# ToyotaResearchInstitute/idto

Measured on AMD Instinct MI355X. Metric: Gauss-Newton iters/sec (grad+Hessian+solve), mini_cheetah N=40, higher is better.
Workload: dtype f64; 1 GPU; mini_cheetah (nq=19, nv=18, 9 contact pairs), horizon N=40, dt=0.05, forward differences, one Gauss-Newton iteration per step; parallelism=single GPU

## Files before the change

idto_amd/csrc/fd_kernel.h:

```cpp
#pragma once

#include "batch.h"
#include "id_eval.h"
#include "id_fast.h"

namespace idto_dev {

struct DevProblem {
  int N;
  double dt;
  const double* v_init;
  const double* q_nom;
  const double* v_nom;
  const double* Qq;
  const double* Qv;
  const double* R;
  const double* Qfq;
  const double* Qfv;
  const double* Qq0; const double* Qv0; const double* R0; const double* Qfq0; const double* Qfv0;
};

__host__ __device__ __forceinline__ DevProblem at_problem(DevProblem P, size_t o) {
  P.v_init = at_problem(P.v_init, o); P.q_nom = at_problem(P.q_nom, o); P.v_nom = at_problem(P.v_nom, o);
  P.Qq = at_problem(P.Qq, o); P.Qv = at_problem(P.Qv, o); P.R = at_problem(P.R, o); P.Qfq = at_problem(P.Qfq, o);
// ... 86 lines not shown
  }
  __syncthreads();
}

IDTO_DEV double velocity_row(const DevModel& M, const double* N, const double* qa, const double* qb, double dt, int r) {
  double acc = N[r] * (qa[0] - qb[0]);
  for (int c = 1; c < M.nq; ++c) acc += N[c * M.nv + r] * (qa[c] - qb[c]);
  return acc / dt;
}
IDTO_DEV void velocity_block(const DevModel& M, const double* N, const double* qa, const double* qb, double dt,
                             double* vout, int tid, int nthreads) {
  for (int r = tid; r < M.nv; r += nthreads) vout[r] = velocity_row(M, N, qa, qb, dt, r);
}

IDTO_DEV double asm_dot(const double* A, const double* B, int nv) {
  const double2* A2 = reinterpret_cast<const double2*>(A);
  const double2* B2 = reinterpret_cast<const double2*>(B);
  double2 a = A2[0], b = B2[0];
  double acc = a.x * b.x;
  if (nv > 1) acc = acc + a.y * b.y;
  const int np = nv >> 1;
#pragma unroll 4
  for (int m = 1; m < np; ++m) {
    a = A2[m]; b = B2[m];
    acc = acc + a.x * b.x;
    acc = acc + a.y * b.y;
  }
  if ((nv & 1) && nv > 1) acc = acc + A[nv - 1] * B[nv - 1];
  return acc;
}
template <int U>
IDTO_DEV void asm_dot_n(const double* const (&A)[U], const double* const (&B)[U], int nv, double (&acc)[U]) {
  const int np = nv >> 1;
#pragma unroll
  for (int u = 0; u < U; ++u) {
    const double2 a = reinterpret_cast<const double2*>(A[u])[0], b = reinterpret_cast<const double2*>(B[u])[0];
    acc[u] = a.x * b.x;
    if (nv > 1) acc[u] = acc[u] + a.y * b.y;
  }
#pragma unroll 2
  for (int m = 1; m < np; ++m) {
#pragma unroll
    for (int u = 0; u < U; ++u) {
      const double2 a = reinterpret_cast<const double2*>(A[u])[m], b = reinterpret_cast<const double2*>(B[u])[m];
      acc[u] = acc[u] + a.x * b.x;
      acc[u] = acc[u] + a.y * b.y;
    }
  }
  if ((nv & 1) && nv > 1) {
#pragma unroll
    for (int u = 0; u < U; ++u) acc[u] = acc[u] + A[u][nv - 1] * B[u][nv - 1];
  }
}
template <int TB>
IDTO_DEV void asm_dot_tile(const double* const (&A)[TB], const double* const (&B)[TB], int nv, double (&acc)[TB][TB]) {
  const int np = nv >> 1;
  double2 a[TB], b[TB];
#pragma unroll
  for (int u = 0; u < TB; ++u) {
    a[u] = reinterpret_cast<const double2*>(A[u])[0];
    b[u] = reinterpret_cast<const double2*>(B[u])[0];
  }
#pragma unroll
  for (int ur = 0; ur < TB; ++ur)
#pragma unroll
    for (int uc = 0; uc < TB; ++uc) {
      acc[ur][uc] = a[ur].x * b[uc].x;
      if (nv > 1) acc[ur][uc] = acc[ur][uc] + a[ur].y * b[uc].y;
    }
  double2 an[TB], bn[TB];
  if (np > 1) {
#pragma unroll
    for (int u = 0; u < TB; ++u) {
      an[u] = reinterpret_cast<const double2*>(A[u])[1];
      bn[u] = reinterpret_cast<const double2*>(B[u])[1];
    }
  }
  for (int m = 1; m < np; ++m) {
#pragma unroll
    for (int u = 0; u < TB; ++u) { a[u] = an[u]; b[u] = bn[u]; }
    const int mn = (m + 1 < np) ? m + 1 : m;
#pragma unroll
    for (int u = 0; u < TB; ++u) {
      an[u] = reinterpret_cast<const double2*>(A[u])[mn];
      bn[u] = reinterpret_cast<const double2*>(B[u])[mn];
    }
#pragma unroll
    for (int ur = 0; ur < TB; ++ur)
#pragma unroll
      for (int uc = 0; uc < TB; ++uc) {
        acc[ur][uc] = acc[ur][uc] + a[ur].x * b[uc].x;
        acc[ur][uc] = acc[ur][uc] + a[ur].y * b[uc].y;
      }
  }
  if ((nv & 1) && nv > 1) {
#pragma unroll
    for (int ur = 0; ur < TB; ++ur)
#pragma unroll
      for (int uc = 0; uc < TB; ++uc) acc[ur][uc] = acc[ur][uc] + A[ur][nv - 1] * B[uc][nv - 1];
  }
}

__host__ __device__ inline int asm_terms_stride(int nq) { return 6 * nq * nq + 3 * nq + ((3 * nq) & 1); }

template <int SHAPE> struct FastShape {
  static constexpr TreeShape T = tree_shape(SHAPE);
  static constexpr int MAXC = T.MAXC, NP = T.NP, CJ = T.CJ, J0 = T.J0, K0 = T.K0, W2 = T.W2, GS = T.GS;
};
__host__ __device__ inline int fd_xch_doubles(int nxb, int threads, int npaths, int nstem = 0) {
  return (threads / npaths) * xch_eval_doubles(nxb, nstem);
}

template <int MAXC, int SHAPE = 0>
IDTO_DEV void fd_body(const DevModel& M, const DevContact& cp, const DevProblem& P, const double* __restrict__ q,
                      double* __restrict__ slab, int slab_stride, double* __restrict__ v_out,
                      double* __restrict__ a_out, double* __restrict__ nplus_out, const int k, int mode,
                      int stop_after, int echunk, double* __restrict__ terms) {
  extern __shared__ double lds[];
  constexpr bool FAST = SHAPE != 0 && SHAPE != SHAPE_XCH && SHAPE != SHAPE_STEM;
  const int tid = threadIdx.x, nt = blockDim.x;
  if (stop_after == 10) return;
#ifdef IDTO_FD_STAMPS
  long long st_arr[16] = {0, 0, 0, 0, 0, 0, 0, 0, 0, 0, 0, 0, 0, 0, 0, 0};
  long long* idto_fd_st = (tid == 0 || tid == IDTO_FD_STAMP_TID) ? st_arr : nullptr;
#endif
  FD_STAMP(0);
  const int nq = M.nq, nv = M.nv, K = M.npaths;
  const int bsz = nv * nq;
  const double dt = P.dt;

  const bool central = mode >= 2;
  const int NM = (mode == 2) ? 2 : ((mode == 3) ? 4 : 1);
  const int nP = (mode >= 1) ? NM * nq : 0;
  const int nT = (mode >= 1) ? NM * nq : 0;
  const int nM = (mode == 1) ? nv : (central ? NM * nq : 0);
  const int E = 1 + nP + nT + nM;

  double* qm1 = lds;
  double* q0 = qm1 + nq;
  double* q1 = q0 + nq;
  double* N0 = q1 + nq;
  double* N1 = N0 + bsz;
  double* v0 = N1 + bsz;
  double* v1 = v0 + nv;
  double* a0 = v1 + nv;
  double* edq = a0 + nv;
  const int EC = (echunk < E) ? echunk : E;
  double* edv = edq + E;
  double* eda = edv + E;
  double* etau = eda + E;
  double* eq = etau + E * nv;
  double* ev = eq + EC * nq;
  double* ea = ev + EC * nv;
  double* edump = ea + EC * nv;
  double* mblob = edump + nv;
  const int blob_lo = FAST ? M.fast_lo : 0, blob_n = FAST ? M.fast_n : M.blob_n;
  int* colinfo = reinterpret_cast<int*>(mblob + blob_n + (blob_n & 1));
  const int nvp = (nv + 1) & ~1, psz = nvp * nq;
  double* rec = reinterpret_cast<double*>(colinfo + nq + (nq & 1));
  rec += (rec - lds) & 1;
  double* xch = rec + (terms ? 6 * psz + nvp : 0);

  const bool sparse = M.nfloat == 0 || (M.nfloat > 0 && nt >= 128);
  const int ql = tid & 63, qcfg = tid >> 6;
  const bool quat_lane = sparse && M.nfloat > 0 && qcfg < 2 && ql >= 48 && ql < 60;
  double qf0[4];
  {
    const double* qq = q + (size_t)(k + (qcfg & 1)) * nq + (M.nfloat > 0 ? M.float_qs[0] : 0);
#pragma unroll
    for (int i = 0; i < 4; ++i) qf0[i] = qq[i];
  }
  double* wr = rec + 6 * psz;
  constexpr int BU = 8;
  double breg[BU];
#pragma unroll
  for (int u = 0; u < BU; ++u) {
    const int i = tid + u * nt;
    breg[u] = (i < blob_n) ? M.blob[blob_lo + i] : 0.0;
  }
  const bool qrow = tid < nq;
  const double g_qm1 = (qrow && k > 0) ? q[(k - 1) * nq + tid] : 0.0;
  const double g_q0 = qrow ? q[k * nq + tid] : 0.0, g_q1 = qrow ? q[(k + 1) * nq + tid] : 0.0;
  const double g_wr = (terms && mode != 0 && tid < nv) ? P.R[tid * nv + tid] : 0.0;
  const double g_nc0 = (sparse && tid < bsz) ? M.nplus_const[tid] : 0.0;
  const double g_nc1 = (sparse && tid + nt < bsz) ? M.nplus_const[tid + nt] : 0.0;
  const int g_ci = (sparse && qrow) ? M.colinfo[tid] : 0;
  const int rowinfo_r = (sparse && tid < nv) ? M.rowinfo[tid] : 0;
  asm volatile("" : "+v"(qf0[0]), "+v"(qf0[1]), "+v"(qf0[2]), "+v"(qf0[3]));
#pragma unroll
  for (int u = 0; u < BU; ++u) {
    const int i = tid + u * nt;
    if (i < blob_n) mblob[i] = breg[u];
  }
  for (int i = tid + BU * nt; i < blob_n; i += nt) mblob[i] = M.blob[blob_lo + i];
  if (qrow) { qm1[tid] = g_qm1; q0[tid] = g_q0; q1[tid] = g_q1; }
  for (int i = tid + nt; i < nq; i += nt) {
    qm1[i] = (k > 0) ? q[(k - 1) * nq + i] : 0.0;
    q0[i] = q[k * nq + i];
    q1[i] = q[(k + 1) * nq + i];
  }
  if (terms && mode != 0) {
    if (tid < nv) wr[tid] = g_wr;
    for (int l = tid + nt; l < nv; l += nt) wr[l] = P.R[l * nv + l];
  }
  if (sparse) {
    if (tid < bsz && g_nc0 == g_nc0) { N0[tid] = g_nc0; N1[tid] = g_nc0; }
    if (tid + nt < bsz && g_nc1 == g_nc1) { N0[tid + nt] = g_nc1; N1[tid + nt] = g_nc1; }
    for (int i = tid + 2 * nt; i < bsz; i += nt) {
      const double cst = M.nplus_const[i];
      if (cst == cst) { N0[i] = cst; N1[i] = cst; }
    }
    if (qrow) colinfo[tid] = g_ci;
    for (int i = tid + nt; i < nq; i += nt) colinfo[i] = M.colinfo[i];
    if (quat_lane) {
      const int e = ql - 48, r = e >> 2, c = e & 3;
      double* Nout = qcfg ? N1 : N0;
      for (int f = 0; f < M.nfloat; ++f) {
        const int qs = M.float_qs[f], vs = M.float_vs[f];
        double qq[4];
#pragma unroll
        for (int i = 0; i < 4; ++i) qq[i] = (f == 0) ? qf0[i] : q[(size_t)(k + qcfg) * nq + qs + i];
        const double nrm = __builtin_sqrt(((qq[0] * qq[0] + qq[1] * qq[1]) + qq[2] * qq[2]) + qq[3] * qq[3]);
        const double t0 = qq[0] / nrm, t1 = qq[1] / nrm, t2 = qq[2] / nrm, t3 = qq[3] / nrm;
        const double w2 = 2.0 * t0, x2 = 2.0 * t1, y2 = 2.0 * t2, z2 = 2.0 * t3;
        const double l0 = (r == 0) ? -x2 : ((r == 1) ? -y2 : -z2);
// ... 149 lines not shown
    using FS = FastShape<SHAPE>;
    FastTab FT;
    FT.body = Ml.f_body; FT.cbody = Ml.f_cbody; FT.pairs = Ml.f_pairs; FT.seg = Ml.f_seg; FT.maxpp = Ml.f_maxpp;
    FT.gslots = Ml.gslots; FT.gcommon = Ml.gcommon;
    const int grp = tid / FS::NP, path = tid % FS::NP;
    for (int e0 = 0; e0 < ce; e0 += groups) {
      const int el = (e0 == 0) ? grp : e0 + (groups - 1 - grp);
      if (el < ce) {
        const bool full = central || c0 + el < 1 + nP + nT;
        if (own_inputs) {
          InFwd in;
          in.q1 = q1; in.v1 = v1; in.a0 = a0; in.N1 = N1; in.N0 = N0; in.nv = nv;
          in.kind = (el == 0) ? 0 : ((el < 1 + nP) ? 1 : ((el < 1 + nP + nT) ? 2 : 3));
          in.col = (el == 0) ? 0 : ((el < 1 + nP) ? el - 1 : ((el < 1 + nP + nT) ? el - 1 - nP : el - 1 - nP - nT));
          in.dq = edq[el];
          in.sdv = (in.kind == 2) ? -edv[el] : ((in.kind == 1) ? edv[el] : 0.0);
          in.sda = (in.kind == 2) ? -eda[el] : ((in.kind == 1) ? eda[el] : 0.0);
          in.keep = (in.kind == 3) ? 0ull : ~0ull;
          in.keep0 = (in.kind == 2) ? ~0ull : 0ull;
          id_eval_fast<FS::MAXC, FS::NP, FS::CJ, FS::J0, FS::K0, FS::W2, FS::GS>(FT, Ml.gravity, cp, path, full, in, etau + el * nv
#ifdef IDTO_FD_STAMPS
                                                                 , (e0 == 0) ? idto_fd_st : nullptr
#endif
          );
        } else {
          InLds in;
          in.q = eq + el * nq; in.v = ev + el * nv; in.a = ea + el * nv;
          id_eval_fast<FS::MAXC, FS::NP, FS::CJ, FS::J0, FS::K0, FS::W2, FS::GS>(FT, Ml.gravity, cp, path, full, in, etau + (c0 + el) * nv);
        }
      }
    }
    if (late_outputs && tid >= nt - 64) trajectory_outputs(tid - (nt - 64), 64);
  } else {
  for (int e0 = 0; e0 < ce; e0 += groups) {
    const int el = e0 + tid / K;
    const int path = tid % K;
    const int ee = (el < ce) ? el : 0;
    const bool full = central || c0 + ee < 1 + nP + nT;
    double* tau_dst = (el < ce) ? etau + (c0 + ee) * nv : edump;
    if constexpr (SHAPE == SHAPE_STEM)
      id_eval<MAXC, true, true>(Ml, cp, path, full, eq + ee * nq, ev + ee * nv, ea + ee * nv, tau_dst,
                                xch + (tid / K) * xch_eval_doubles(Ml.nxb, Ml.nstem));
    else if constexpr (SHAPE == SHAPE_XCH)
      id_eval<MAXC, true>(Ml, cp, path, full, eq + ee * nq, ev + ee * nv, ea + ee * nv, tau_dst, xch + (tid / K) * Ml.nxb * XREC);
    else
      id_eval<MAXC>(Ml, cp, path, full, eq + ee * nq, ev + ee * nv, ea + ee * nv, tau_dst);
  }
  }
  __syncthreads();
  }

  FD_STAMP(12);
  if (stop_after == 3) return;
  double* sl = slab + (size_t)k * slab_stride;
  double* Mk = sl;
  double* Tk = sl + bsz;
  double* Pk = sl + 2 * bsz;
  double* tauk = sl + 3 * bsz;
  for (int r = tid; r < nv; r += nt) tauk[r] = etau[r];
  if (mode == 1) {
    const double sc = 1 / dt / dt;
    const double* Mcols = etau + (1 + nP + nT) * nv;
    const double fillM = (k == 0) ? __builtin_nan("") : 0.0;
    constexpr int RU = 2;
    for (int base = tid; base < bsz; base += RU * nt) {
      int ii[RU], rr[RU], j0[RU], cnt[RU];
      bool ok[RU];
      double tp[RU], tt[RU], t0[RU], dqp[RU], dqt[RU], w[RU], mc[RU][3], n0[RU][3];
#pragma unroll
      for (int u = 0; u < RU; ++u) {
        const int idx = base + u * nt;
        ok[u] = idx < bsz;
        const int id = ok[u] ? idx : 0;
        ii[u] = id / nv; rr[u] = id - ii[u] * nv;
        const int ci = colinfo[ii[u]];
        j0[u] = ci & 0xffff; cnt[u] = ci >> 16;
        tp[u] = etau[(1 + ii[u]) * nv + rr[u]]; tt[u] = etau[(1 + nP + ii[u]) * nv + rr[u]]; t0[u] = etau[rr[u]];
        dqp[u] = edq[1 + ii[u]]; dqt[u] = edq[1 + nP + ii[u]];
        w[u] = terms ? wr[rr[u]] : 0.0;
#pragma unroll
        for (int t = 0; t < 3; ++t) {
          const int j = (t < cnt[u]) ? j0[u] + t : j0[u];
          mc[u][t] = Mcols[j * nv + rr[u]];
          n0[u][t] = N0[ii[u] * nv + j];
        }
      }
#pragma unroll
      for (int u = 0; u < RU; ++u) {
        if (!ok[u]) continue;
        const int idx = base + u * nt, i = ii[u], r = rr[u];
        const double pv = (tp[u] - t0[u]) / dqp[u];
        const double tv = (k >= 1) ? (tt[u] - t0[u]) / dqt[u] : 0.0;
        double acc = (sc * mc[u][0]) * n0[u][0];
        if (cnt[u] > 1) acc += (sc * mc[u][1]) * n0[u][1];
        if (cnt[u] > 2) acc += (sc * mc[u][2]) * n0[u][2];
        const double mv = (k >= 2) ? acc : fillM;
        Pk[idx] = pv;
        Tk[idx] = tv;
        Mk[idx] = mv;
        if (terms) {
          const double mr = (k >= 2) ? acc : 0.0;
          rec[i * nvp + r] = pv; rec[psz + i * nvp + r] = tv; rec[2 * psz + i * nvp + r] = mr;
          rec[3 * psz + i * nvp + r] = pv * w[u]; rec[4 * psz + i * nvp + r] = tv * w[u]; rec[5 * psz + i * nvp + r] = mr * w[u];
          if (r == nv - 1 && nvp > nv) {
            rec[3 * psz + i * nvp + nv] = 0.0; rec[4 * psz + i * nvp + nv] = 0.0; rec[5 * psz + i * nvp + nv] = 0.0;
          }
        }
      }
    }
  } else if (central) {
    for (int idx = tid; idx < 3 * bsz; idx += nt) {
      const int g = idx / bsz, rem = idx - g * bsz, i = rem / nv, r = rem - i * nv;
      const int e0 = 1 + (g * NM) * nq + i;
      const double dq = edq[e0];
      const double tp = etau[e0 * nv + r], tm = etau[(e0 + nq) * nv + r];
      double d;
      if (mode == 2) {
        d = 0.5 * (tp - tm) / dq;
      } else {
        const double tpp = etau[(e0 + 2 * nq) * nv + r], tmm = etau[(e0 + 3 * nq) * nv + r];
        d = 2.0 / 3.0 * (tp - tm) / dq - 1.0 / 12.0 * (tpp - tmm) / dq;
      }
      const double val = (g == 0) ? d : ((g == 1) ? ((k >= 1) ? d : 0.0) : ((k >= 2) ? d : ((k == 0) ? __builtin_nan("") : 0.0)));
      if (g == 0) Pk[rem] = val;
      else if (g == 1) Tk[rem] = val;
      else Mk[rem] = val;
      if (terms) {
        const double rv = (g == 2 && k < 2) ? 0.0 : val;
        rec[g * psz + i * nvp + r] = rv;
        rec[(3 + g) * psz + i * nvp + r] = rv * wr[r];
        if (r == nv - 1 && nvp > nv) rec[(3 + g) * psz + i * nvp + nv] = 0.0;
      }
    }
  }
  if (!terms || mode == 0 || stop_after == 4) return;
  FD_STAMP(13);
  __syncthreads();
  if (stop_after == 5) return;
  const int qq = nq * nq, ts = asm_terms_stride(nq);
  double* stage = terms + (size_t)k * ts;
  constexpr int TB = 3;
  const int nb = (nq + TB - 1) / TB, ntt = nb * (nb + 1) / 2, nbb = nb * nb, ntiles = 3 * ntt + 3 * nbb;
  const float inb = 1.0f / (float)nb;
  for (int tile = tid; tile < ntiles; tile += nt) {
    if (stop_after == 6 && tile >= 3 * ntt) break;
    int xa, sb, tr, tc, ob;
    const bool lower = tile < 3 * ntt;
    if (lower) {
      const int which = (tile >= ntt) + (tile >= 2 * ntt);
      int rem = tile - which * ntt;
      tc = 0;
      while (rem >= nb - tc) { rem -= nb - tc; ++tc; }
      tr = tc + rem;
      xa = which; sb = which; ob = which * qq;
    } else {
      const int it = tile - 3 * ntt, which = (it >= nbb) + (it >= 2 * nbb), e = it - which * nbb;
      tc = (int)(((float)e + 0.5f) * inb);
      tr = e - tc * nb;
      xa = (which == 1) ? 1 : 0; sb = (which == 0) ? 1 : 2; ob = (3 + which) * qq;
    }
    const double* A[TB];
    const double* B[TB];
#pragma unroll
    for (int u = 0; u < TB; ++u) {
      const int r = tr * TB + u, c = tc * TB + u;
      A[u] = rec + (3 + xa) * psz + (r < nq ? r : nq - 1) * nvp;
      B[u] = rec + sb * psz + (c < nq ? c : nq - 1) * nvp;
    }
    double acc[TB][TB];
    asm_dot_tile<TB>(A, B, nv, acc);
#pragma unroll
    for (int ur = 0; ur < TB; ++ur)
#pragma unroll
      for (int uc = 0; uc < TB; ++uc) {
        const int r = tr * TB + ur, c = tc * TB + uc;
        if (r < nq && c < nq && (!lower || r >= c)) stage[ob + c * nq + r] = acc[ur][uc];
      }
  }
  if (stop_after != 7)
    for (int it = nt - 1 - tid; it < 3 * nq; it += nt) {
      const int which = (it >= nq) + (it >= 2 * nq), j = it - which * nq;
      const double* J = rec + which * psz + j * nvp;
      double acc = (etau[0] * wr[0]) * J[0];
      for (int r = 1; r < nv; ++r) acc += (etau[r] * wr[r]) * J[r];
      stage[6 * qq + which * nq + j] = acc;
    }
  FD_STAMP(14);
  FD_STAMP(15);
#ifdef IDTO_FD_STAMPS
  if (idto_fd_st && k == 1)
    for (int i = 0; i < 16; ++i) nplus_out[(size_t)(k + 1) * bsz + (tid == 0 ? 0 : 16) + i] = (double)(st_arr[i] - st_arr[0]);
#endif
}

template <int MAXC, int SHAPE = 0>
__global__ void __launch_bounds__(256) fd_kernel(DevModel M, DevContact cp, DevProblem P, const double* __restrict__ q,
                          double* __restrict__ slab, int slab_stride, double* __restrict__ v_out,
                          double* __restrict__ a_out, double* __restrict__ nplus_out, int k_begin, int mode,
                          int stop_after, int echunk, size_t pstride, double* __restrict__ terms, AltSel alt) {
  const size_t o = (size_t)blockIdx.y * pstride;
  const size_t w = o + (size_t)alt_offset(alt, o);
  fd_body<MAXC, SHAPE>(M, cp, at_problem(P, o), at_problem(q, o), at_problem(slab, w), slab_stride, at_problem(v_out, w),
                       at_problem(a_out, w), at_problem(nplus_out, w), k_begin + (int)blockIdx.x, mode, stop_after, echunk,
                       terms ? at_problem(terms, w) : nullptr);
}


}
```

idto_amd/csrc/host/model_tables.cc:

```cpp
#include "model_tables.h"

#include <algorithm>
#include <cmath>
#include <cstring>
#include <limits>

#include "model_layout.h"

namespace idto_host {
namespace {
using namespace idto_dev;

int Refuse(std::string* err, const char* why) {
  *err = why;
  return -1;
}

bool IdentityRotation(const double* X) {
  bool ident = true;
  for (int e = 0; e < 9; ++e) ident &= (X[e] == ((e % 4 == 0) ? 1.0 : 0.0));
  return ident;
}

int CheckGeometry(const idto_model_t* m, std::string* err) {
// ... 188 lines not shown
  std::vector<int> colinfo, rowinfo;
  int nfloat = 0, float_qs[4] = {0, 0, 0, 0}, float_vs[4] = {0, 0, 0, 0};
};
NPlus BuildNPlus(const idto_model_t* m) {
  const int nq = m->nq, nv = m->nv;
  NPlus n;
  n.constant.assign((size_t)nv * nq, 0.0);
  n.colinfo.assign(nq, 0);
  n.rowinfo.assign(nv, 0);
  auto one = [&](int q, int v) { n.constant[(size_t)q * nv + v] = 1.0; n.colinfo[q] = v | 1 << 16; n.rowinfo[v] = q | 1 << 16; };
  for (int b = 0; b < m->nbodies; ++b) {
    const int qs = m->qstart[b], vs = m->vstart[b], jt = m->jtype[b];
    if (jt == IDTO_JOINT_REVOLUTE || jt == IDTO_JOINT_PRISMATIC) {
      one(qs, vs);
    } else if (jt == IDTO_JOINT_PLANAR) {
      for (int k = 0; k < 3; ++k) one(qs + k, vs + k);
    } else {
      for (int r = 0; r < 3; ++r)
        for (int cq = 0; cq < 4; ++cq) n.constant[(size_t)(qs + cq) * nv + vs + r] = std::numeric_limits<double>::quiet_NaN();
      for (int k = 0; k < 4; ++k) n.colinfo[qs + k] = vs | 3 << 16;
      for (int r = 0; r < 3; ++r) n.rowinfo[vs + r] = qs | 4 << 16;
      for (int k = 0; k < 3; ++k) one(qs + 4 + k, vs + 3 + k);
      if (n.nfloat >= 0 && n.nfloat < 4) { n.float_qs[n.nfloat] = qs; n.float_vs[n.nfloat] = vs; ++n.nfloat; }
      else n.nfloat = -1;
    }
  }
  return n;
}

struct FastShapeOf {
  int shape = 0;
  int w2 = -1;
};
FastShapeOf RecogniseShape(const idto_model_t* m, const Stem& stem, const Star& star, bool shared, bool capsules) {
  const int K = m->npaths, cbody = m->common_body, cj = cbody >= 0 ? m->jtype[cbody] : -1;
  FastShapeOf f;
  bool ok = !(cbody >= 0 && cj != IDTO_JOINT_FLOATING) && !shared && stem.n() <= 1 && !capsules;
  for (int p = 0; p < K; ++p) ok = ok && star.nchain[p] == star.maxc;
  int j0 = -1, k0 = -1;
  for (int p = 0; p < K && ok; ++p)
    for (int s = 0; s < star.maxc; ++s) {
      const int jt = m->jtype[star.chain[star.at(p, s)]], kd = star.pkind[star.at(p, s)];
      if (s == 0) {
        if (p == 0) { j0 = jt; k0 = kd; }
        if (jt != j0 || kd != k0) ok = false;
      } else if (jt == IDTO_JOINT_REVOLUTE && kd == PK_WORLD && K == 1 && f.w2 < 0) {
        f.w2 = s;
      } else if (jt != IDTO_JOINT_REVOLUTE || kd != PK_PREV) {
        ok = false;
      }
    }
  for (int s = 1; s <= kNumTreeShapes && ok; ++s) {
    const TreeShape& t = kTreeShapes[s - 1];
    if (star.maxc == t.MAXC && K == t.NP && cj == t.CJ && j0 == t.J0 && k0 == t.K0 && f.w2 == t.W2 && (t.GS || star.all_gravity))
      f.shape = s;
  }
  return f;
}

struct FastOrder {
  std::vector<std::vector<int>> order;
  std::vector<int> seg;
};
FastOrder OrderFastPairs(const idto_model_t* m, const Star& star, const PairLists& l, FastShapeOf* f) {
  const int K = m->npaths, maxc = star.maxc, w2 = f->w2;
  const std::vector<int>&sa = l.sa, &sb = l.sb;
  FastOrder o;
  o.order.resize(K);
  o.seg.assign((size_t)K * (maxc + 2), 0);
  for (int p = 0; p < K && f->shape; ++p) {
    const int* first = l.path_pairs.data() + (size_t)p * l.maxpp;
    const std::vector<int> mine(first, first + l.path_npairs[p]);
    int lo_chain_common = 1 << 30, hi_chain_common = -1, last_slot = -1;
    for (int pi : mine) {
      const int nchainb = (sa[pi] >= 0) + (sb[pi] >= 0);
      if (nchainb > 1) {
        bool fine = w2 >= 0 && std::min(sa[pi], sb[pi]) == w2 - 1 && std::max(sa[pi], sb[pi]) == w2;
        for (int pj : mine) fine = fine && (pj == pi || (sa[pj] != w2 - 1 && sb[pj] != w2 - 1));
        if (!fine) { f->shape = 0; break; }
        continue;
      }
      if (nchainb == 1 && (sa[pi] == -1 || sb[pi] == -1)) {
        const int sl = std::max(sa[pi], sb[pi]);
        if (sl < last_slot) { f->shape = 0; break; }
        last_slot = sl;
        lo_chain_common = std::min(lo_chain_common, pi);
        hi_chain_common = std::max(hi_chain_common, pi);
      }
    }
    if (!f->shape) break;
    std::vector<std::vector<int>> groups(maxc + 2);
    for (int pi : mine) {
      const int sl = std::max(sa[pi], sb[pi]);
      if (sl >= 0) { groups[1 + sl].push_back(pi); continue; }
      const bool touches_common = sa[pi] == -1 || sb[pi] == -1;
      if (!touches_common || (sa[pi] == -1 && sb[pi] == -1)) { f->shape = 0; break; }
      if (pi < lo_chain_common) groups[0].push_back(pi);
      else if (pi > hi_chain_common) groups[maxc + 1].push_back(pi);
      else { f->shape = 0; break; }
    }
    if (!f->shape) break;
    for (int gi = 0; gi < maxc + 2; ++gi) {
      o.seg[(size_t)p * (maxc + 2) + gi] = (int)o.order[p].size() | ((int)groups[gi].size() << 16);
      for (int pi : groups[gi]) o.order[p].push_back(pi);
    }
  }
  return o;
// ... 125 lines not shown
```

idto_amd/csrc/id_fast.h:

```cpp
#pragma once

#include "id_eval.h"

#ifdef IDTO_FD_STAMPS
#ifndef IDTO_FD_STAMP_TID
#define IDTO_FD_STAMP_TID 192
#endif
#define FD_STAMP(i) do { __builtin_amdgcn_sched_barrier(0); asm volatile("" ::: "memory"); if (idto_fd_st) idto_fd_st[i] = (long long)__builtin_readcyclecounter(); asm volatile("" ::: "memory"); __builtin_amdgcn_sched_barrier(0); } while (0)
#else
#define FD_STAMP(i) do { } while (0)
#endif

namespace idto_dev {

template <int CTRL>
IDTO_DEV double quad_perm(double x) {
  int lo = __double2loint(x), hi = __double2hiint(x);
  lo = __builtin_amdgcn_update_dpp(0, lo, CTRL, 0xf, 0xf, true);
  hi = __builtin_amdgcn_update_dpp(0, hi, CTRL, 0xf, 0xf, true);
  return __hiloint2double(hi, lo);
}
template <int NP>
IDTO_DEV V3 tree_sum_fast(V3 v) {
  if (NP >= 2) {
    v.x = v.x + quad_perm<0xB1>(v.x); v.y = v.y + quad_perm<0xB1>(v.y); v.z = v.z + quad_perm<0xB1>(v.z);
  }
  if (NP >= 4) {
    v.x = v.x + quad_perm<0x4E>(v.x); v.y = v.y + quad_perm<0x4E>(v.y); v.z = v.z + quad_perm<0x4E>(v.z);
  }
  if (NP >= 8) {
    v.x = xor_add(v.x, 4); v.y = xor_add(v.y, 4); v.z = xor_add(v.z, 4);
  }
  return v;
}

IDTO_DEV const double* lds_launder(const double* p) {
  typedef __attribute__((address_space(3))) const double lds_cdouble;
  unsigned a = (unsigned)(size_t)(lds_cdouble*)p;
  asm volatile("" : "+v"(a));
  return (const double*)(lds_cdouble*)(size_t)a;
}

IDTO_DEV void pin(V3& a) { asm volatile("" : "+v"(a.x), "+v"(a.y), "+v"(a.z)); }

enum { FB_PREFETCH = FB_INERTIA + 6 };
IDTO_DEV void prefetch_record(const double* rec, double (&rc)[FB_PREFETCH]) {
#ifdef IDTO_FAST_NO_PREFETCH
#pragma unroll
  for (int i = 0; i < FB_PREFETCH; ++i) rc[i] = rec[i];
#else
  typedef __attribute__((address_space(3))) const volatile double lds_cvdouble;
  lds_cvdouble* p = (lds_cvdouble*)rec;
#pragma unroll
  for (int i = 0; i < FB_PREFETCH; ++i) rc[i] = p[i];
#endif
}

struct ParentKin {
  M3 R;
  V3 p, w, v, al, a;
// ... 397 lines not shown
```

idto_amd/csrc/idto_hip.hip:

```cpp
#include <hip/hip_runtime.h>
#include <rccl/rccl.h>
#include <dlfcn.h>

#include <atomic>
#include <chrono>
#include <cmath>
#include <cstdio>
#include <cstdlib>
#include <cstring>
#include <initializer_list>
#include <limits>
#include <memory>
#include <mutex>
#include <type_traits>
#include <utility>
#include <thread>
#include <string>
#include <vector>

#include "idto_hip.h"
#include "kernels.h"
#include "fd_launch.h"
#include "penta_ldl.h"
#include "fused.h"
// ... 390 lines not shown
      HIP_OK(hipStreamSynchronize(c->stream));
      TRACE("hip: problem upload done (one copy + wait)");
    }
  }
  auto is_diag = [](const double* W, int n) {
    for (int c2 = 0; c2 < n; ++c2)
      for (int r = 0; r < n; ++r)
        if (r != c2 && W[(size_t)c2 * n + r] != 0.0) return false;
    return true;
  };
  const bool diag = is_diag(p->Qq, nq) && is_diag(p->Qv, nv) && is_diag(p->R, nv) && is_diag(p->Qf_q, nq) &&
                    is_diag(p->Qf_v, nv);
  if ((int)c->prob_diag.size() != c->batch) c->prob_diag.assign((size_t)c->batch, 0);
  c->prob_diag[(size_t)pb] = diag ? 1 : 0;
  c->weights_diagonal = true;
  for (char d : c->prob_diag) c->weights_diagonal = c->weights_diagonal && d;
  DevProblem& P = c->P;
  P.N = N; P.dt = dt; P.v_init = c->d_vinit; P.q_nom = c->d_qnom; P.v_nom = c->d_vnom;
  P.Qq = c->d_w[0]; P.Qv = c->d_w[1]; P.R = c->d_w[2]; P.Qfq = c->d_w[3]; P.Qfv = c->d_w[4];
  P.Qq0 = c->d_w[5]; P.Qv0 = c->d_w[6]; P.R0 = c->d_w[7]; P.Qfq0 = c->d_w[8]; P.Qfv0 = c->d_w[9];
  return 0;
}

int UploadModel(idto_hip_ctx* c, const idto_model_t* m, const idto_host::ModelTables& t) {
  double* bd = nullptr;
  if (Upload(c, t.blob.data(), t.blob.size(), &bd)) return -2;
  const int* bi = reinterpret_cast<const int*>(bd);
  DevModel& M = c->M;
  M.blob = bd; M.blob_n = (int)t.blob.size();
#define X(name) M.name = bd + t.at.name;
  IDTO_MODEL_DOUBLE_TABLES(X)
#undef X
#define X(name) M.name = bi + t.at.name;
  IDTO_MODEL_INT_TABLES(X)
#undef X
  M.nb = m->nbodies; M.nq = m->nq; M.nv = m->nv; M.npaths = m->npaths; M.common_body = m->common_body;
  M.ngeoms = m->ngeoms; M.npairs = m->npairs; M.maxpp = t.maxpp;
  for (int i = 0; i < 3; ++i) M.gravity[i] = m->gravity[i];
  M.nfloat = t.nfloat;
  for (int i = 0; i < 4; ++i) { M.float_qs[i] = t.float_qs[i]; M.float_vs[i] = t.float_vs[i]; }
  M.fast_shape = t.fast_shape; M.fast_lo = t.fast_lo; M.fast_n = t.fast_n; M.f_maxpp = t.f_maxpp;
  M.gslots = t.gslots; M.gcommon = t.gcommon; M.gstem = t.gstem; M.nxb = t.nxb; M.nstem = t.nstem;
  c->maxc = t.maxc; c->capsules = t.capsules;
  return 0;
}


int FdEvals(const idto_hip_ctx* c, int mode) {
  return (mode == 0) ? 1 : ((mode == 1) ? 1 + 2 * c->nq + c->nv : 1 + ((mode == 2) ? 2 : 4) * 3 * c->nq);
}

int FdLds(const idto_hip_ctx* c, int mode, int ec, bool with_terms = false, bool fast = true, int threads = 0) {
  const int nq = c->nq, nv = c->nv, E = FdEvals(c, mode), nvp = (nv + 1) & ~1;
  const int rec = with_terms ? 6 * nvp * nq + nvp + 1 : 0;
  const int blob_n = (fast && c->fd_fast && c->M.fast_shape) ? c->M.fast_n : c->M.blob_n;
  if (!threads) threads = mode >= 1 ? c->fd_threads : 64;
  const int xch = fd_xch_doubles(c->M.nxb, threads, c->npaths, c->M.nstem);
  return (int)sizeof(double) * (3 * nq + 2 * nv * nq + 3 * nv + 3 * E + E * nv + ec * (nq + 2 * nv) + nv + blob_n + 2 + nq / 2 + 2 + rec + xch);
}

static int FdBlock(const idto_hip_ctx* c, int mode) {
  if (mode == 0) return 64;
  int t = c->fd_threads;
  while (c->M.nstem > 1 && t > 64 && FdLds(c, mode, t / c->npaths, false, true, t) > 160 * 1024) t -= 64;
  return t;
}

static bool FoldTerms(const idto_hip_ctx* c, int mode) { return c->asm_fold && c->weights_diagonal && mode >= 1; }

int LaunchFd(idto_hip_ctx* c, int mode, int kb, int ke, AltSel alt = AltSel{nullptr, 0, 0}) {
  c->partials_ahead = false;
  if (ke <= kb) return 0;
  if (mode >= 1) mode = 1 + c->gradients_method;
  dim3 grid(ke - kb, c->batch), block(FdBlock(c, mode));
  const int E = FdEvals(c, mode), groups = (int)block.x / c->npaths;
  int ec = E;
  bool fold = FoldTerms(c, mode);
  if (fold && FdLds(c, mode, std::min(ec, groups), true, true, block.x) > 160 * 1024) fold = false;
  while (ec > groups && FdLds(c, mode, ec, fold, true, block.x) > 160 * 1024) ec = ((ec - 1) / groups) * groups;
  const int lds = FdLds(c, mode, ec, fold, true, block.x);
  if (lds > 160 * 1024) { g_err = "finite-difference evaluation set does not fit in LDS"; return -1; }
  double* terms = fold ? c->terms : nullptr;
  if (mode >= 1) c->terms_valid = fold && kb == 0 && ke == c->N;
  FdLaunch fl;
  fl.grid = grid; fl.block = block; fl.lds = lds; fl.stream = c->stream; fl.M = c->M; fl.cp = c->cp; fl.P = c->P;
  fl.q = c->q; fl.slab = c->slab; fl.slab_stride = c->slab_stride; fl.v = c->v; fl.a = c->a; fl.nplus = c->nplus;
  fl.k_begin = kb; fl.mode = mode; fl.stop_after = c->fd_stop; fl.echunk = ec; fl.pstride = c->pstride; fl.terms = terms;
  fl.alt = alt;
  fl.shape = c->fd_fast ? c->M.fast_shape : 0;
  if (c->M.nxb) fl.shape = SHAPE_XCH;
  if (c->M.nstem > 1) fl.shape = SHAPE_STEM;
  fl.maxc = c->maxc;
  fd_launch(fl);
  HIP_OK(hipGetLastError());
  return 0;
}

int TimeBegin(idto_hip_ctx* c, int which) {
  c->timing_open = false;
  if (!c->timing) return 0;
  if ((c->timing_tick[which]++ % (unsigned)c->timing_stride) != 0) return 0;
  c->timing_open = true;
  idto_hip_ctx::Timed t;
  t.which = which;
  hipEvent_t* ev[2] = {&t.a, &t.b};
  for (hipEvent_t* e : ev) {
    if (c->event_pool.empty()) {
// ... 2246 lines not shown
```

idto_amd/csrc/model_layout.h:

```cpp
#pragma once

#include "idto_model.h"

namespace idto_dev {

enum { PK_WORLD = 0, PK_COMMON = 1, PK_PREV = 2 };

enum { FB_XPF = 0, FB_AXIS = 12, FB_MASS = 15, FB_COM = 16, FB_INERTIA = 19, FB_DAMP = 25, FB_IDX = 31, FB_STRIDE = 34 };
enum { FP_INFO = 0, FP_XC = 2, FP_SC = 14, FP_XO = 17, FP_SO = 29, FP_STRIDE = 34 };

struct TreeShape { int MAXC, NP, CJ, J0, K0, W2, GS, KC; };
constexpr TreeShape kTreeShapes[] = {
    {2, 1, -1, IDTO_JOINT_REVOLUTE, PK_WORLD, -1, 0, 2},
    {3, 1, -1, IDTO_JOINT_PLANAR, PK_WORLD, -1, 0, 3},
    {3, 4, IDTO_JOINT_FLOATING, IDTO_JOINT_REVOLUTE, PK_COMMON, -1, 0, 3},
    {4, 4, IDTO_JOINT_FLOATING, IDTO_JOINT_REVOLUTE, PK_WORLD, -1, 0, 4},
    {3, 1, -1, IDTO_JOINT_REVOLUTE, PK_WORLD, 2, 0, 3},
    {7, 1, IDTO_JOINT_FLOATING, IDTO_JOINT_REVOLUTE, PK_WORLD, -1, 1, 8},
};
constexpr int kNumTreeShapes = sizeof(kTreeShapes) / sizeof(kTreeShapes[0]);
constexpr int SHAPE_XCH = kNumTreeShapes + 1;
constexpr int SHAPE_STEM = kNumTreeShapes + 2;
constexpr TreeShape tree_shape(int shape) {
  return shape >= 1 && shape <= kNumTreeShapes ? kTreeShapes[shape - 1] : TreeShape{0, 1, -1, 0, 0, -1, 0, 8};
}

}
```

Measured before the change: 12660 GN iters/s.

## Specialize FD Hessian-term assembly on compile-time model sizes and fold gradient into tiles

Derives nq/nv at compile time for the known tree shapes and uses them throughout the finite-difference term assembly, so loops fully unroll and index math becomes constant. The dot-tile routine gains a fully unrolled path that preloads all operand pairs. The separate gradient-term loop is removed: a weighted tau row is stored in LDS and used as an extra tile row, so the gradient comes out of the same tile pass. The cost is a bit more LDS, more registers in the unrolled tile, and a stricter shape match that now requires nq/nv to agree.

```diff
diff --git a/idto_amd/csrc/fd_kernel.h b/idto_amd/csrc/fd_kernel.h
--- a/idto_amd/csrc/fd_kernel.h
+++ b/idto_amd/csrc/fd_kernel.h
@@ -162,8 +162,47 @@
     for (int u = 0; u < U; ++u) acc[u] = acc[u] + A[u][nv - 1] * B[u][nv - 1];
   }
 }
-template <int TB>
-IDTO_DEV void asm_dot_tile(const double* const (&A)[TB], const double* const (&B)[TB], int nv, double (&acc)[TB][TB]) {
+template <int TB, int NV = 0>
+IDTO_DEV void asm_dot_tile(const double* const (&A)[TB], const double* const (&B)[TB], int nv, double (&acc)[TB][TB]
+#ifdef IDTO_FD_STAMPS
+                           , long long* idto_fd_st = nullptr
+#endif
+) {
+  if constexpr (NV > 1) {
+    constexpr int NP = NV >> 1;
+    double2 a[NP][TB], b[NP][TB];
+#pragma unroll
+    for (int m = 0; m < NP; ++m)
+#pragma unroll
+      for (int u = 0; u < TB; ++u) {
+        a[m][u] = reinterpret_cast<const double2*>(A[u])[m];
+        b[m][u] = reinterpret_cast<const double2*>(B[u])[m];
+      }
+#pragma unroll
+    for (int m = 0; m < NP; ++m) {
+#pragma unroll
+      for (int ur = 0; ur < TB; ++ur)
+#pragma unroll
+        for (int uc = 0; uc < TB; ++uc) {
+          if (m == 0) acc[ur][uc] = a[m][ur].x * b[m][uc].x;
+          else acc[ur][uc] = acc[ur][uc] + a[m][ur].x * b[m][uc].x;
+          acc[ur][uc] = acc[ur][uc] + a[m][ur].y * b[m][uc].y;
+        }
+#pragma unroll
+      for (int ur = 0; ur < TB; ++ur)
+#pragma unroll
+        for (int uc = 0; uc < TB; ++uc) asm volatile("" : "+v"(acc[ur][uc]));
+      if (m == 0) FD_STAMP(18);
+    }
+    if (NV & 1) {
+#pragma unroll
+      for (int ur = 0; ur < TB; ++ur)
+#pragma unroll
+        for (int uc = 0; uc < TB; ++uc) acc[ur][uc] = acc[ur][uc] + A[ur][NV - 1] * B[uc][NV - 1];
+    }
+    FD_STAMP(19);
+    return;
+  }
   const int np = nv >> 1;
   double2 a[TB], b[TB];
 #pragma unroll
@@ -178,6 +217,7 @@
       acc[ur][uc] = a[ur].x * b[uc].x;
       if (nv > 1) acc[ur][uc] = acc[ur][uc] + a[ur].y * b[uc].y;
     }
+  FD_STAMP(18);
   double2 an[TB], bn[TB];
   if (np > 1) {
 #pragma unroll
@@ -209,6 +249,7 @@
 #pragma unroll
       for (int uc = 0; uc < TB; ++uc) acc[ur][uc] = acc[ur][uc] + A[ur][nv - 1] * B[uc][nv - 1];
   }
+  FD_STAMP(19);
 }
 
 __host__ __device__ inline int asm_terms_stride(int nq) { return 6 * nq * nq + 3 * nq + ((3 * nq) & 1); }
@@ -231,7 +272,7 @@
   const int tid = threadIdx.x, nt = blockDim.x;
   if (stop_after == 10) return;
 #ifdef IDTO_FD_STAMPS
-  long long st_arr[16] = {0, 0, 0, 0, 0, 0, 0, 0, 0, 0, 0, 0, 0, 0, 0, 0};
+  long long st_arr[IDTO_FD_NSTAMPS] = {};
   long long* idto_fd_st = (tid == 0 || tid == IDTO_FD_STAMP_TID) ? st_arr : nullptr;
 #endif
   FD_STAMP(0);
@@ -269,7 +310,7 @@
   const int nvp = (nv + 1) & ~1, psz = nvp * nq;
   double* rec = reinterpret_cast<double*>(colinfo + nq + (nq & 1));
   rec += (rec - lds) & 1;
-  double* xch = rec + (terms ? 6 * psz + nvp : 0);
+  double* xch = rec + (terms ? 6 * psz + 2 * nvp : 0);
 
   const bool sparse = M.nfloat == 0 || (M.nfloat > 0 && nt >= 128);
   const int ql = tid & 63, qcfg = tid >> 6;
@@ -281,6 +322,7 @@
     for (int i = 0; i < 4; ++i) qf0[i] = qq[i];
   }
   double* wr = rec + 6 * psz;
+  double* tw = wr + nvp;
   constexpr int BU = 8;
   double breg[BU];
 #pragma unroll
@@ -536,73 +578,89 @@
 
   FD_STAMP(12);
   if (stop_after == 3) return;
+  constexpr bool GROWS = FAST;
+  constexpr bool CSIZES = FAST && SHAPE <= kNumSizedShapes;
+  constexpr int CNQ = CSIZES ? tree_shape_nq(SHAPE) : 0, CNV = CSIZES ? tree_shape_nv(SHAPE) : 0, CNVP = (CNV + 1) & ~1;
+  const int tnq = CNQ ? CNQ : nq, tnv = CNQ ? CNV : nv, tbsz = CNQ ? CNV * CNQ : bsz, tnvp = CNQ ? CNVP : nvp, tpsz = CNQ ? CNVP * CNQ : psz;
   double* sl = slab + (size_t)k * slab_stride;
   double* Mk = sl;
-  double* Tk = sl + bsz;
-  double* Pk = sl + 2 * bsz;
-  double* tauk = sl + 3 * bsz;
-  for (int r = tid; r < nv; r += nt) tauk[r] = etau[r];
+  double* Tk = sl + tbsz;
+  double* Pk = sl + 2 * tbsz;
+  double* tauk = sl + 3 * tbsz;
+  for (int r = tid; r < tnv; r += nt) tauk[r] = etau[r];
+  if constexpr (GROWS)
+    if (terms && mode != 0)
+      for (int r = nt - 1 - tid; r < tnvp; r += nt) tw[r] = (r < tnv) ? etau[r] * wr[r] : 0.0;
   if (mode == 1) {
     const double sc = 1 / dt / dt;
-    const double* Mcols = etau + (1 + nP + nT) * nv;
+    const double* Mcols = etau + (1 + tnq + tnq) * tnv;
     const double fillM = (k == 0) ? __builtin_nan("") : 0.0;
     constexpr int RU = 2;
-    for (int base = tid; base < bsz; base += RU * nt) {
+    for (int base = tid; base < tbsz; base += RU * nt) {
       int ii[RU], rr[RU], j0[RU], cnt[RU];
       bool ok[RU];
       double tp[RU], tt[RU], t0[RU], dqp[RU], dqt[RU], w[RU], mc[RU][3], n0[RU][3];
 #pragma unroll
       for (int u = 0; u < RU; ++u) {
         const int idx = base + u * nt;
-        ok[u] = idx < bsz;
+        ok[u] = idx < tbsz;
         const int id = ok[u] ? idx : 0;
-        ii[u] = id / nv; rr[u] = id - ii[u] * nv;
+        ii[u] = id / tnv; rr[u] = id - ii[u] * tnv;
         const int ci = colinfo[ii[u]];
         j0[u] = ci & 0xffff; cnt[u] = ci >> 16;
-        tp[u] = etau[(1 + ii[u]) * nv + rr[u]]; tt[u] = etau[(1 + nP + ii[u]) * nv + rr[u]]; t0[u] = etau[rr[u]];
-        dqp[u] = edq[1 + ii[u]]; dqt[u] = edq[1 + nP + ii[u]];
+        tp[u] = etau[(1 + ii[u]) * tnv + rr[u]]; tt[u] = etau[(1 + tnq + ii[u]) * tnv + rr[u]]; t0[u] = etau[rr[u]];
+        dqp[u] = edq[1 + ii[u]]; dqt[u] = edq[1 + tnq + ii[u]];
         w[u] = terms ? wr[rr[u]] : 0.0;
 #pragma unroll
         for (int t = 0; t < 3; ++t) {
           const int j = (t < cnt[u]) ? j0[u] + t : j0[u];
-          mc[u][t] = Mcols[j * nv + rr[u]];
-          n0[u][t] = N0[ii[u] * nv + j];
+          mc[u][t] = Mcols[j * tnv + rr[u]];
+          n0[u][t] = N0[ii[u] * tnv + j];
         }
       }
+      FD_STAMP(13);
+      double pvs[RU], tvs[RU], accs[RU];
+#pragma unroll
+      for (int u = 0; u < RU; ++u) {
+        if (!ok[u]) continue;
+        pvs[u] = (tp[u] - t0[u]) / dqp[u];
+        tvs[u] = (k >= 1) ? (tt[u] - t0[u]) / dqt[u] : 0.0;
+        double acc = (sc * mc[u][0]) * n0[u][0];
+        if (cnt[u] > 1) acc += (sc * mc[u][1]) * n0[u][1];
+        if (cnt[u] > 2) acc += (sc * mc[u][2]) * n0[u][2];
+        accs[u] = acc;
+      }
+      FD_STAMP(14);
 #pragma unroll
       for (int u = 0; u < RU; ++u) {
         if (!ok[u]) continue;
         const int idx = base + u * nt, i = ii[u], r = rr[u];
-        const double pv = (tp[u] - t0[u]) / dqp[u];
-        const double tv = (k >= 1) ? (tt[u] - t0[u]) / dqt[u] : 0.0;
-        double acc = (sc * mc[u][0]) * n0[u][0];
-        if (cnt[u] > 1) acc += (sc * mc[u][1]) * n0[u][1];
-        if (cnt[u] > 2) acc += (sc * mc[u][2]) * n0[u][2];
+        const double pv = pvs[u], tv = tvs[u], acc = accs[u];
         const double mv = (k >= 2) ? acc : fillM;
         Pk[idx] = pv;
         Tk[idx] = tv;
         Mk[idx] = mv;
         if (terms) {
           const double mr = (k >= 2) ? acc : 0.0;
-          rec[i * nvp + r] = pv; rec[psz + i * nvp + r] = tv; rec[2 * psz + i * nvp + r] = mr;
-          rec[3 * psz + i * nvp + r] = pv * w[u]; rec[4 * psz + i * nvp + r] = tv * w[u]; rec[5 * psz + i * nvp + r] = mr * w[u];
-          if (r == nv - 1 && nvp > nv) {
-            rec[3 * psz + i * nvp + nv] = 0.0; rec[4 * psz + i * nvp + nv] = 0.0; rec[5 * psz + i * nvp + nv] = 0.0;
+          rec[i * tnvp + r] = pv; rec[tpsz + i * tnvp + r] = tv; rec[2 * tpsz + i * tnvp + r] = mr;
+          rec[3 * tpsz + i * tnvp + r] = pv * w[u]; rec[4 * tpsz + i * tnvp + r] = tv * w[u]; rec[5 * tpsz + i * tnvp + r] = mr * w[u];
+          if (r == tnv - 1 && tnvp > tnv) {
+            rec[3 * tpsz + i * tnvp + tnv] = 0.0; rec[4 * tpsz + i * tnvp + tnv] = 0.0; rec[5 * tpsz + i * tnvp + tnv] = 0.0;
           }
         }
       }
     }
   } else if (central) {
-    for (int idx = tid; idx < 3 * bsz; idx += nt) {
-      const int g = idx / bsz, rem = idx - g * bsz, i = rem / nv, r = rem - i * nv;
-      const int e0 = 1 + (g * NM) * nq + i;
+    for (int idx = tid; idx < 3 * tbsz; idx += nt) {
+      const int g = idx / tbsz, rem = idx - g * tbsz, i = rem / tnv, r = rem - i * tnv;
+      const int e0 = 1 + (g * NM) * tnq + i;
       const double dq = edq[e0];
-      const double tp = etau[e0 * nv + r], tm = etau[(e0 + nq) * nv + r];
+      const double tp = etau[e0 * tnv + r], tm = etau[(e0 + tnq) * tnv + r];
       double d;
       if (mode == 2) {
         d = 0.5 * (tp - tm) / dq;
       } else {
-        const double tpp = etau[(e0 + 2 * nq) * nv + r], tmm = etau[(e0 + 3 * nq) * nv + r];
+        const double tpp = etau[(e0 + 2 * tnq) * tnv + r], tmm = etau[(e0 + 3 * tnq) * tnv + r];
         d = 2.0 / 3.0 * (tp - tm) / dq - 1.0 / 12.0 * (tpp - tmm) / dq;
       }
       const double val = (g == 0) ? d : ((g == 1) ? ((k >= 1) ? d : 0.0) : ((k >= 2) ? d : ((k == 0) ? __builtin_nan("") : 0.0)));
@@ -611,20 +669,21 @@
       else Mk[rem] = val;
       if (terms) {
         const double rv = (g == 2 && k < 2) ? 0.0 : val;
-        rec[g * psz + i * nvp + r] = rv;
-        rec[(3 + g) * psz + i * nvp + r] = rv * wr[r];
-        if (r == nv - 1 && nvp > nv) rec[(3 + g) * psz + i * nvp + nv] = 0.0;
+        rec[g * tpsz + i * tnvp + r] = rv;
+        rec[(3 + g) * tpsz + i * tnvp + r] = rv * wr[r];
+        if (r == tnv - 1 && tnvp > tnv) rec[(3 + g) * tpsz + i * tnvp + tnv] = 0.0;
       }
     }
   }
   if (!terms || mode == 0 || stop_after == 4) return;
-  FD_STAMP(13);
+  FD_STAMP(15);
   __syncthreads();
+  FD_STAMP(16);
   if (stop_after == 5) return;
-  const int qq = nq * nq, ts = asm_terms_stride(nq);
+  const int qq = tnq * tnq, ts = asm_terms_stride(tnq);
   double* stage = terms + (size_t)k * ts;
   constexpr int TB = 3;
-  const int nb = (nq + TB - 1) / TB, ntt = nb * (nb + 1) / 2, nbb = nb * nb, ntiles = 3 * ntt + 3 * nbb;
+  const int nb = (tnq + TB - 1) / TB, nbr = GROWS ? tnq / TB + 1 : nb, ntt = nb * nbr - nb * (nb - 1) / 2, nbb = nb * nb, ntiles = 3 * ntt + 3 * nbb;
   const float inb = 1.0f / (float)nb;
   for (int tile = tid; tile < ntiles; tile += nt) {
     if (stop_after == 6 && tile >= 3 * ntt) break;
@@ -634,12 +693,25 @@
       const int which = (tile >= ntt) + (tile >= 2 * ntt);
       int rem = tile - which * ntt;
       tc = 0;
-      while (rem >= nb - tc) { rem -= nb - tc; ++tc; }
+      if constexpr (CNQ != 0) {
+        constexpr int NB = (CNQ + TB - 1) / TB, NBR = CNQ / TB + 1;
+        int off = 0;
+#pragma unroll
+        for (int t = 0, S = 0; t < NB - 1; ++t) {
+          S += NBR - t;
+          const bool ge = rem >= S;
+          tc += ge; off = ge ? S : off;
+        }
+        rem -= off;
+      } else {
+        while (rem >= nbr - tc) { rem -= nbr - tc; ++tc; }
+      }
       tr = tc + rem;
       xa = which; sb = which; ob = which * qq;
     } else {
       const int it = tile - 3 * ntt, which = (it >= nbb) + (it >= 2 * nbb), e = it - which * nbb;
-      tc = (int)(((float)e + 0.5f) * inb);
+      if constexpr (CNQ != 0) tc = e / nb;
+      else tc = (int)(((float)e + 0.5f) * inb);
       tr = e - tc * nb;
       xa = (which == 1) ? 1 : 0; sb = (which == 0) ? 1 : 2; ob = (3 + which) * qq;
     }
@@ -648,32 +720,43 @@
 #pragma unroll
     for (int u = 0; u < TB; ++u) {
       const int r = tr * TB + u, c = tc * TB + u;
-      A[u] = rec + (3 + xa) * psz + (r < nq ? r : nq - 1) * nvp;
-      B[u] = rec + sb * psz + (c < nq ? c : nq - 1) * nvp;
+      if constexpr (GROWS) A[u] = r < tnq ? rec + (3 + xa) * tpsz + r * tnvp : tw;
+      else A[u] = rec + (3 + xa) * tpsz + (r < tnq ? r : tnq - 1) * tnvp;
+      B[u] = rec + sb * tpsz + (c < tnq ? c : tnq - 1) * tnvp;
     }
     double acc[TB][TB];
-    asm_dot_tile<TB>(A, B, nv, acc);
+    FD_STAMP(17);
+#ifdef IDTO_FD_STAMPS
+    asm_dot_tile<TB, CNV>(A, B, tnv, acc, idto_fd_st);
+#else
+    asm_dot_tile<TB, CNV>(A, B, tnv, acc);
+#endif
 #pragma unroll
     for (int ur = 0; ur < TB; ++ur)
 #pragma unroll
       for (int uc = 0; uc < TB; ++uc) {
         const int r = tr * TB + ur, c = tc * TB + uc;
-        if (r < nq && c < nq && (!lower || r >= c)) stage[ob + c * nq + r] = acc[ur][uc];
-      }
-  }
-  if (stop_after != 7)
-    for (int it = nt - 1 - tid; it < 3 * nq; it += nt) {
-      const int which = (it >= nq) + (it >= 2 * nq), j = it - which * nq;
-      const double* J = rec + which * psz + j * nvp;
-      double acc = (etau[0] * wr[0]) * J[0];
-      for (int r = 1; r < nv; ++r) acc += (etau[r] * wr[r]) * J[r];
-      stage[6 * qq + which * nq + j] = acc;
-    }
-  FD_STAMP(14);
-  FD_STAMP(15);
+        if (r < tnq && c < tnq && (!lower || r >= c)) stage[ob + c * tnq + r] = acc[ur][uc];
+        if constexpr (GROWS)
+          if (lower && r == tnq && c < tnq && stop_after != 7) stage[6 * qq + xa * tnq + c] = acc[ur][uc];
+      }
+    FD_STAMP(20);
+  }
+  FD_STAMP(21);
+  if constexpr (!GROWS)
+    if (stop_after != 7)
+      for (int it = nt - 1 - tid; it < 3 * tnq; it += nt) {
+        const int which = (it >= tnq) + (it >= 2 * tnq), j = it - which * tnq;
+        const double* J = rec + which * tpsz + j * tnvp;
+        double acc = (etau[0] * wr[0]) * J[0];
+        for (int r = 1; r < tnv; ++r) acc += (etau[r] * wr[r]) * J[r];
+        stage[6 * qq + which * tnq + j] = acc;
+      }
+  FD_STAMP(22);
 #ifdef IDTO_FD_STAMPS
-  if (idto_fd_st && k == 1)
-    for (int i = 0; i < 16; ++i) nplus_out[(size_t)(k + 1) * bsz + (tid == 0 ? 0 : 16) + i] = (double)(st_arr[i] - st_arr[0]);
+  if (idto_fd_st && k == 1 && 2 * IDTO_FD_NSTAMPS <= tbsz)
+    for (int i = 0; i < IDTO_FD_NSTAMPS; ++i)
+      nplus_out[(size_t)(k + 1) * tbsz + (tid == 0 ? 0 : IDTO_FD_NSTAMPS) + i] = (double)(st_arr[i] - st_arr[0]);
 #endif
 }
 
diff --git a/idto_amd/csrc/host/model_tables.cc b/idto_amd/csrc/host/model_tables.cc
--- a/idto_amd/csrc/host/model_tables.cc
+++ b/idto_amd/csrc/host/model_tables.cc
@@ -264,7 +264,8 @@
     }
   for (int s = 1; s <= kNumTreeShapes && ok; ++s) {
     const TreeShape& t = kTreeShapes[s - 1];
-    if (star.maxc == t.MAXC && K == t.NP && cj == t.CJ && j0 == t.J0 && k0 == t.K0 && f.w2 == t.W2 && (t.GS || star.all_gravity))
+    if (star.maxc == t.MAXC && K == t.NP && cj == t.CJ && j0 == t.J0 && k0 == t.K0 && f.w2 == t.W2 && (t.GS || star.all_gravity) &&
+        m->nq == tree_shape_nq(s) && m->nv == tree_shape_nv(s))
       f.shape = s;
   }
   return f;
diff --git a/idto_amd/csrc/id_fast.h b/idto_amd/csrc/id_fast.h
--- a/idto_amd/csrc/id_fast.h
+++ b/idto_amd/csrc/id_fast.h
@@ -6,6 +6,7 @@
 #ifndef IDTO_FD_STAMP_TID
 #define IDTO_FD_STAMP_TID 192
 #endif
+#define IDTO_FD_NSTAMPS 24
 #define FD_STAMP(i) do { __builtin_amdgcn_sched_barrier(0); asm volatile("" ::: "memory"); if (idto_fd_st) idto_fd_st[i] = (long long)__builtin_readcyclecounter(); asm volatile("" ::: "memory"); __builtin_amdgcn_sched_barrier(0); } while (0)
 #else
 #define FD_STAMP(i) do { } while (0)
diff --git a/idto_amd/csrc/idto_hip.hip b/idto_amd/csrc/idto_hip.hip
--- a/idto_amd/csrc/idto_hip.hip
+++ b/idto_amd/csrc/idto_hip.hip
@@ -466,7 +466,7 @@
 
 int FdLds(const idto_hip_ctx* c, int mode, int ec, bool with_terms = false, bool fast = true, int threads = 0) {
   const int nq = c->nq, nv = c->nv, E = FdEvals(c, mode), nvp = (nv + 1) & ~1;
-  const int rec = with_terms ? 6 * nvp * nq + nvp + 1 : 0;
+  const int rec = with_terms ? 6 * nvp * nq + 2 * nvp + 1 : 0;
   const int blob_n = (fast && c->fd_fast && c->M.fast_shape) ? c->M.fast_n : c->M.blob_n;
   if (!threads) threads = mode >= 1 ? c->fd_threads : 64;
   const int xch = fd_xch_doubles(c->M.nxb, threads, c->npaths, c->M.nstem);
diff --git a/idto_amd/csrc/model_layout.h b/idto_amd/csrc/model_layout.h
--- a/idto_amd/csrc/model_layout.h
+++ b/idto_amd/csrc/model_layout.h
@@ -24,5 +24,24 @@
 constexpr TreeShape tree_shape(int shape) {
   return shape >= 1 && shape <= kNumTreeShapes ? kTreeShapes[shape - 1] : TreeShape{0, 1, -1, 0, 0, -1, 0, 8};
 }
+constexpr int kNumSizedShapes = 5;
+constexpr int joint_nq(int jt) { return jt == IDTO_JOINT_FLOATING ? 7 : (jt == IDTO_JOINT_PLANAR ? 3 : (jt < 0 ? 0 : 1)); }
+constexpr int joint_nv(int jt) { return jt == IDTO_JOINT_FLOATING ? 6 : (jt == IDTO_JOINT_PLANAR ? 3 : (jt < 0 ? 0 : 1)); }
+constexpr int tree_shape_nq(int shape) {
+  return shape >= 1 && shape <= kNumTreeShapes
+             ? joint_nq(kTreeShapes[shape - 1].CJ) + kTreeShapes[shape - 1].NP * (joint_nq(kTreeShapes[shape - 1].J0) + kTreeShapes[shape - 1].MAXC - 1)
+             : 0;
+}
+constexpr int tree_shape_nv(int shape) {
+  return shape >= 1 && shape <= kNumTreeShapes
+             ? joint_nv(kTreeShapes[shape - 1].CJ) + kTreeShapes[shape - 1].NP * (joint_nv(kTreeShapes[shape - 1].J0) + kTreeShapes[shape - 1].MAXC - 1)
+             : 0;
+}
+static_assert(tree_shape_nq(1) == 2 && tree_shape_nv(1) == 2, "acrobot");
+static_assert(tree_shape_nq(2) == 5 && tree_shape_nv(2) == 5, "hopper");
+static_assert(tree_shape_nq(3) == 19 && tree_shape_nv(3) == 18, "mini_cheetah");
+static_assert(tree_shape_nq(4) == 23 && tree_shape_nv(4) == 22, "allegro_hand");
+static_assert(tree_shape_nq(5) == 3 && tree_shape_nv(5) == 3, "spinner");
+static_assert(tree_shape_nq(6) == 14 && tree_shape_nv(6) == 13, "jaco, jaco_ball");
 
 }
```

After: 13020 GN iters/s (median of 6 runs). 2.9% higher.
